# gergely-flamich/compression-without-quantization

Hardware: AMD Instinct MI355X
Metric: latent blocks encoded/s at KL=16 bits (higher is better)
Workload: dtype f32

## Files before the change

### compression_without_quantization_amd/csrc/cwq_kernels.hip

```cpp
#include <hip/hip_runtime.h>

#include <type_traits>
#include <stdint.h>

#include "cwq_device.h"
#include "cwq_kernels.h"

namespace cwq {

__global__ void __launch_bounds__(256) k_prep_dims(
    const float* __restrict__ t_scale, const float* __restrict__ p_loc,
    const float* __restrict__ p_scale, int64_t n, float nst, float sdiv, float rho,
    float* __restrict__ loc_s, float* __restrict__ scale_s, float* __restrict__ lognorm,
    float* __restrict__ out_sample, unsigned long long* __restrict__ keys, int64_t nb) {
  for (int64_t g = blockIdx.x * (int64_t)blockDim.x + threadIdx.x; g < nb;
       g += (int64_t)gridDim.x * blockDim.x)
    keys[g] = 0ull;
  for (int64_t i = blockIdx.x * (int64_t)blockDim.x + threadIdx.x; i < n;
       i += (int64_t)gridDim.x * blockDim.x) {
    float ls, ss;
    shard_consts(p_loc[i], p_scale[i], nst, sdiv, rho, ls, ss);
    loc_s[i] = ls;
    scale_s[i] = ss;
    lognorm[i] = lognorm_of(t_scale[i]);
    out_sample[i] = 0.0f;
  }
}

template <int DC, bool STEP0>
__device__ __forceinline__ float eval_row(const PhiloxStream& st, uint64_t kbase, int64_t d_rt,
                                          int align_rt, const float* __restrict__ loc_s,
                                          const float* __restrict__ scale_s,
                                          const float* __restrict__ mu,
                                          const float* __restrict__ sg,
                                          const float* __restrict__ lognorm,
                                          const float* __restrict__ best,
                                          const double* logtab) {
  return eval_row_f<DC>(st, kbase, d_rt, align_rt, logtab, [&](int64_t e, float zz) -> float {
    float s = scale_s[e] * zz;
    s = loc_s[e] + s;
    const float tv = STEP0 ? s : best[e] + s;
    return log_prob(tv, mu[e], sg[e], lognorm[e]);
  });
}

template <int DC, bool STEP0>
__global__ void __launch_bounds__(256) k_encode_eval(
    const float* __restrict__ t_loc, const float* __restrict__ t_scale,
    const float* __restrict__ loc_s, const float* __restrict__ scale_s,
    const float* __restrict__ lognorm, const float* __restrict__ best,
    const int64_t* __restrict__ block_off, int64_t ud, int64_t ntiles, int64_t tiles_per_block,
    int64_t cand_per_tile, int64_t n_cand, SeedSpec sd, int32_t step,
    unsigned long long* __restrict__ keys) {
  __shared__ double logtab[32];
  __shared__ unsigned long long wkey[4];
  fill_logtab(logtab);
  const uint32_t wv = wave_id();
  const uint32_t lane = threadIdx.x & 63u;

  for (int64_t tile = blockIdx.x; tile < ntiles; tile += gridDim.x) {
    const int64_t g = tile / tiles_per_block;
    const int64_t tt = tile - g * tiles_per_block;
    const BlockSpan sp = block_span(block_off, ud, g);
    const int64_t n0 = tt * cand_per_tile;
    const int64_t n1 = (n0 + cand_per_tile < n_cand) ? n0 + cand_per_tile : n_cand;
    const PhiloxStream st =
        generate_key(step_seed(sd.of(g), step), 42);
    const int align = (int)(((uint64_t)(n0 + wv) * (uint64_t)sp.d) & 3u);

    uint64_t bestk = 0;
    for (int64_t n = n0 + 4 * (int64_t)lane + wv; n < n1; n += 256) {
      const float v = eval_row<DC, STEP0>(st, (uint64_t)n * (uint64_t)sp.d, sp.d, align,
                                          loc_s + sp.off, scale_s + sp.off, t_loc + sp.off,
                                          t_scale + sp.off, lognorm + sp.off,
                                          STEP0 ? nullptr : best + sp.off, logtab);
      const uint64_t k = argmax_key(v, (uint32_t)n);
      bestk = k > bestk ? k : bestk;
    }
    bestk = wave_max_u64(bestk);
    if (lane == 0) wkey[wv] = bestk;
    __syncthreads();
    if (threadIdx.x == 0) {
      uint64_t m = wkey[0];
      for (int i = 1; i < 4; ++i) m = wkey[i] > m ? wkey[i] : m;
      if (m) atomicMax(&keys[g], (unsigned long long)m);
    }
    __syncthreads();
  }
}

constexpr float kPruneC1 = 0x1p-14f;
#ifndef CWQ_PRUNE_MIN_WAVES
#define CWQ_PRUNE_MIN_WAVES 6
#endif
#ifndef CWQ_XCD_BALANCE
#define CWQ_XCD_BALANCE 1
#endif
#ifndef CWQ_TAU_SHARE_MASK
#define CWQ_TAU_SHARE_MASK 15u
#endif
#ifndef CWQ_SURVIVOR_CAP
#define CWQ_SURVIVOR_CAP 1024
#endif

template <bool STEP0>
__device__ __forceinline__ float cand_diff(float z, float ls, float ss, float mu, float bb) {
  const float s = shard_sample(ls, ss, z);
  const float tv = STEP0 ? s : bb + s;
  return tv - mu;
}
__device__ __forceinline__ float lp_from_z(float z, float cc) {
  const float u = -0.5f * (z * z);
  return u - cc;
}


#ifdef CWQ_TILE_TIMES
constexpr int kTileTimes = 1 << 18;
__device__ unsigned long long g_tile_t0[kTileTimes], g_tile_t1[kTileTimes];
__device__ unsigned int g_tile_wg[kTileTimes];
#endif
#ifdef CWQ_PRUNE_STATS
__device__ unsigned long long g_prune_stats[72];
constexpr int kDbgBlocks = 1 << 20;
__device__ unsigned long long g_dbg_best[kDbgBlocks];
__device__ int g_seed_tau;
#endif

template <int D, bool STEP0, bool INTER>
__global__ void __launch_bounds__(256, CWQ_PRUNE_MIN_WAVES) k_encode_prune(
    const float* __restrict__ t_loc, const float* __restrict__ t_scale,
    const float* __restrict__ loc_s, const float* __restrict__ scale_s,
    const float* __restrict__ lognorm, const float* __restrict__ best, int64_t ntiles,
    int64_t tiles_per_block, int64_t cand_per_tile, int64_t n_cand, SeedSpec sd, int32_t step,
    int allow_screen, unsigned long long* __restrict__ keys, int64_t tail_from, int tail_div,
    uint32_t* __restrict__ tq) {
  static_assert(D % 8 == 0 && D >= 8 && D <= 64, "pruned path: D % 8 == 0, D <= 64");
  constexpr int G = D / 4;
  constexpr int NF = STEP0 ? 6 : 7;
  constexpr int NS = 2;
  __shared__ double logtab[32];
  __shared__ float4 cst[G * NF];
  __shared__ float4 scst[G * NS];
  __shared__ int2 meta[G];
  __shared__ float dscore[D];
  __shared__ float dA[D];
  __shared__ float dC[D];
  __shared__ float gscore[G];
  __shared__ int gpos[G];
  __shared__ float lowc;
  __shared__ float scr_a, scr_pq;
  __shared__ uint32_t tau_ord;
  __shared__ uint32_t sq_cnt;
  __shared__ uint32_t sq_n[CWQ_SURVIVOR_CAP];
  __shared__ float sq_ub[CWQ_SURVIVOR_CAP];
  __shared__ unsigned long long wkey[4];
  __shared__ uint32_t s_next;
#ifdef CWQ_PRUNE_STATS
  __shared__ uint32_t s_ps[72];
  for (int i = threadIdx.x; i < 72; i += blockDim.x) s_ps[i] = 0u;
#endif
  fill_logtab(logtab);
  const uint32_t wv = wave_id();
  const uint32_t lane = threadIdx.x & 63u;

  constexpr bool inter = INTER;
  const int64_t nbt = INTER ? ntiles / tiles_per_block : 0;
  auto next_tile = [&](int64_t cur) -> int64_t {
    if (tq == nullptr) return cur + gridDim.x;
    __syncthreads();
    if (threadIdx.x == 0) s_next = gridDim.x + atomicAdd(tq, 1u);
    __syncthreads();
    return (int64_t)s_next;
  };
  for (int64_t tile = blockIdx.x; tile < ntiles; tile = next_tile(tile)) {
    uint32_t tid = threadIdx.x;
    asm volatile("" : "+v"(tid));
#ifdef CWQ_TILE_TIMES
    if (tid == 0 && tile < kTileTimes) {
      g_tile_t0[tile] = __builtin_amdgcn_s_memrealtime();
      const uint32_t xcc = (uint32_t)__builtin_amdgcn_s_getreg((20) | (0 << 6) | ((4 - 1) << 11));
      g_tile_wg[tile] = (xcc << 24) | (blockIdx.x & 0xffffffu);
    }
#endif
    int64_t tord = tile;
    const int64_t treg = inter ? nbt * tail_from : 0;
    if (inter && CWQ_XCD_BALANCE && tq == nullptr && tile < treg && (treg & 7) == 0 &&
        (gridDim.x & 7u) == 0)
      tord = (tile & 7) * (treg >> 3) + (tile >> 3);
    const int64_t g = inter ? tord % nbt : tile / tiles_per_block;
    const int64_t tt = inter ? tord / nbt : tile - g * tiles_per_block;
    const int64_t off = g * D;
    int64_t n0, csz;
    if (tt < tail_from) {
      n0 = tt * cand_per_tile;
      csz = cand_per_tile;
    } else {
      csz = cand_per_tile / tail_div;
      n0 = tail_from * cand_per_tile + (tt - tail_from) * csz;
    }
    const int64_t n1 = (n0 + csz < n_cand) ? n0 + csz : n_cand;
    if (n0 >= n1) continue;
    const PhiloxStream st =
        generate_key(step_seed(sd.of(g), step), 42);

    if (tid < D) {
      const int j = tid;
      const float ls = loc_s[off + j], ss = scale_s[off + j], mu = t_loc[off + j];
      const float rs = 1.0f / t_scale[off + j];
      const float m = (STEP0 ? ls : best[off + j] + ls) - mu;
      float e = 0.5f * (ss * ss + m * m) * (rs * rs);
      dscore[j] = (e == e) ? e : -1.0f;
    }
    __syncthreads();
    if (tid < G) {
      const int q = tid;
      gscore[q] = ((dscore[4 * q] + dscore[4 * q + 1]) + dscore[4 * q + 2]) + dscore[4 * q + 3];
    }
    __syncthreads();
    if (tid < G) {
      const int q = tid;
      const float sq = gscore[q];
      int r = 0;
      for (int q2 = 0; q2 < G; ++q2) {
        const float s2 = gscore[q2];
        r += (s2 > sq || (s2 == sq && q2 < q)) ? 1 : 0;
      }
      gpos[q] = r;
      meta[r].x = q;
    }
    __syncthreads();
    int den_ok = 1, scr_ok = 1;
    if (tid < D) {
      const int j = tid, k = gpos[j >> 2], w = j & 3;
      float fj[7];
      const float sgj = t_scale[off + j];
      fj[0] = loc_s[off + j];
      fj[1] = scale_s[off + j];
      fj[2] = t_loc[off + j];
      fj[3] = sgj;
      fj[4] = lognorm[off + j];
      fj[5] = 1.0f / sgj;
      fj[6] = STEP0 ? 0.0f : best[off + j];
      float* c = reinterpret_cast<float*>(cst);
#pragma unroll
      for (int f = 0; f < NF; ++f) c[(k * NF + f) * 4 + w] = fj[f];
      den_ok = markstein_ok_den(sgj) ? 1 : 0;
      const ScreenDim o = screen_dim<STEP0>(fj[0], fj[1], fj[2], sgj, fj[4], fj[6]);
      float* sc = reinterpret_cast<float*>(scst);
      sc[(k * NS + 0) * 4 + w] = o.sa;
      sc[(k * NS + 1) * 4 + w] = o.sb;
      dA[j] = o.A;
      dC[j] = o.C;
      scr_ok = o.ok ? 1 : 0;
    }
    const bool fastdiv = __syncthreads_and(den_ok) != 0;
    const bool scr_all = __syncthreads_and(scr_ok) != 0;
    const bool screen = allow_screen && scr_all;
    if (tid <= G + 1) {
      const int kb = tid;
      const float* c = reinterpret_cast<const float*>(cst);
      double rf = 0.0, kk = 0.0, asum = 0.0, msum = 0.0, kall = 0.0, cvis = 0.0, a2 = 0.0,
             amax = 0.0;
#pragma unroll 1
      for (int p = 0; p < D; ++p) {
        const double mj = -(double)c[((p >> 2) * NF + 4) * 4 + (p & 3)];
        const double aj = __builtin_fabs(mj);
        asum += aj;
        msum += mj;
        kall += aj + mj;
        if (p >= 4 * kb) {
          rf += mj + 0x1p-17 * aj;
        } else {
          kk += aj + mj;
          if (screen) cvis += (double)dC[(meta[p >> 2].x << 2) + (p & 3)];
        }
        if (screen && kb == G + 1) {
          const double av = (double)dA[p];
          a2 += av * av;
          amax = av > amax ? av : amax;
        }
      }
      const double marg = 0x1p-20 * (__builtin_fabs(rf) + asum) + 0x1p-126;
      const double sl = 0x1p-14 * (__builtin_fabs(msum) + asum + kall) + 0x1p-126;
      if (kb <= G) {
        const float bk = screen ? round_up_f32(msum + cvis * (1.0 + 0x1p-20) + sl)
                                : round_up_f32(rf + 0x1p-14 * kk + marg);
        if (kb >= 1) meta[kb - 1].y = (int)f2u(bk);
        if (kb == G) lowc = round_up_f32(0x1p-14 * kk + marg);
      } else if (screen) {
        scr_a = screen_as(msum, sl, a2);
        scr_pq = screen_pq(amax, D);
      }
      if (kb == 0) {
        uint32_t t0 = ord_f32(-__builtin_inff());
        if (inter) {
          const unsigned long long kv =
              __hip_atomic_load(&keys[g], __ATOMIC_RELAXED, __HIP_MEMORY_SCOPE_AGENT);
          if ((uint32_t)(kv >> 32) > kArgmaxClampOrd) t0 = (uint32_t)(kv >> 32);
        }
        tau_ord = t0;
#ifdef CWQ_PRUNE_STATS
        if (g_seed_tau && g < kDbgBlocks && (g_dbg_best[g] >> 32) > kArgmaxClampOrd)
          tau_ord = (uint32_t)(g_dbg_best[g] >> 32);
#endif
        sq_cnt = 0u;
      }
    }
    __syncthreads();
    const float lc = lowc;
#ifdef CWQ_PRUNE_STATS
    const float tau_seed = unord_f32(tau_ord);
#endif
    const float sA = scr_a, sPq = scr_pq;

    const int64_t per_wave = (n1 - n0 + 3) / 4;
    const int64_t w0 = n0 + (int64_t)wv * per_wave;
    const uint32_t w1 = (uint32_t)((w0 + per_wave < n1) ? w0 + per_wave : n1);
    uint32_t wnext = (uint32_t)w0 + 64u;
    uint32_t n = (uint32_t)w0 + lane;
    int k = 0;
    float s = 0.0f;
#ifndef CWQ_TAU_FROM_KEYS
#define CWQ_TAU_FROM_KEYS 1
#endif
    float tau = (INTER && CWQ_TAU_FROM_KEYS) ? unord_f32(tau_ord) : -__builtin_inff();
#ifdef CWQ_PRUNE_STATS
    tau = tau_seed;
#endif
    uint64_t bestk = 0;
    uint32_t iter = 0;

    const PhiloxLo lok = philox_lo_key(st);
    auto pass = [&](auto screen_tag) {
      constexpr bool SCREEN = decltype(screen_tag)::value;
      for (;;) {
        const bool active = n < w1;
        if (__ballot(active) == 0ull) break;
        const int2 mt = meta[k];
        const uint32_t grp = (uint32_t)n * (uint32_t)G + (uint32_t)mt.x;
        const U4 x = philox10_lo(grp, lok, st.k0, st.k1);
        float z0, z1, z2, z3;
        float upper;
        if constexpr (SCREEN) {
          box_muller_screen(x.x, x.y, z0, z1);
          box_muller_screen(x.z, x.w, z2, z3);
          const float4* cq = scst + k * NS;
          const float4 sa = cq[0], sb = cq[1];
          const float a0 = __builtin_fmaf(sa.x, z0, sb.x);
          const float a1 = __builtin_fmaf(sa.y, z1, sb.y);
          const float a2 = __builtin_fmaf(sa.z, z2, sb.z);
          const float a3 = __builtin_fmaf(sa.w, z3, sb.w);
          s = __builtin_fmaf(-a0, a0, s);
          s = __builtin_fmaf(-a1, a1, s);
          s = __builtin_fmaf(-a2, a2, s);
          s = __builtin_fmaf(-a3, a3, s);
          upper = screen_row_upper(s, kScreenC1, u2f((uint32_t)mt.y));
        } else {
          box_muller_dev(x.x, x.y, logtab, z0, z1);
          box_muller_dev(x.z, x.w, logtab, z2, z3);
          const float4* cq = cst + k * NF;
          const float4 ls = cq[0], ss = cq[1], mu = cq[2], sg = cq[3], cc = cq[4], ry = cq[5];
          const float4 bb = STEP0 ? float4{0.f, 0.f, 0.f, 0.f} : cq[6];
          const float d0 = cand_diff<STEP0>(z0, ls.x, ss.x, mu.x, bb.x);
          const float d1 = cand_diff<STEP0>(z1, ls.y, ss.y, mu.y, bb.y);
          const float d2 = cand_diff<STEP0>(z2, ls.z, ss.z, mu.z, bb.z);
          const float d3 = cand_diff<STEP0>(z3, ls.w, ss.w, mu.w, bb.w);
          float y0 = div_rn_markstein(d0, sg.x, ry.x);
          float y1 = div_rn_markstein(d1, sg.y, ry.y);
          float y2 = div_rn_markstein(d2, sg.z, ry.z);
          float y3 = div_rn_markstein(d3, sg.w, ry.w);
          const bool ok = fastdiv & markstein_ok4(d0, d1, d2, d3);
          if (__builtin_expect(__ballot(!ok) != 0ull, 0)) {
            if (!ok) {
              y0 = d0 / sg.x;
              y1 = d1 / sg.y;
              y2 = d2 / sg.z;
              y3 = d3 / sg.w;
            }
          }
          s = s + lp_from_z(y0, cc.x);
          s = s + lp_from_z(y1, cc.y);
          s = s + lp_from_z(y2, cc.z);
          s = s + lp_from_z(y3, cc.w);
          upper = (s + __builtin_fabsf(s) * kPruneC1) + u2f((uint32_t)mt.y);
        }
        k += 1;
        const bool complete = (k == G);
        const bool below = upper < tau;
#ifdef CWQ_PRUNE_STATS
        const bool prune = !complete && below;
#endif
        const bool done = complete || below || !active;
        const uint64_t m = __ballot(complete) | __ballot(below) |
                           (__builtin_amdgcn_read_exec() & ~__ballot(active));
        if (complete && active && upper >= tau) {
          float lower;
          if constexpr (SCREEN)
            lower = screen_row_lower(s, kScreenC2, sA, sPq);
          else
            lower = (s - __builtin_fabsf(s) * kPruneC1) - lc;
          tau = fmaxf(tau, lower);
          const uint32_t slot = atomicAdd(&sq_cnt, 1u);
          if (slot < CWQ_SURVIVOR_CAP) {
            sq_n[slot] = (uint32_t)n;
            sq_ub[slot] = upper;
          } else {
#ifdef CWQ_PRUNE_STATS
            atomicAdd(&g_prune_stats[69], 1ull);
#endif
            const float v = eval_row<D, STEP0>(st, (uint64_t)n * D, D, 0, loc_s + off,
                                               scale_s + off, t_loc + off, t_scale + off,
                                               lognorm + off, STEP0 ? nullptr : best + off, logtab);
            const uint64_t kv = argmax_key(v, (uint32_t)n);
            bestk = kv > bestk ? kv : bestk;
          }
        }
#ifdef CWQ_PRUNE_STATS
        if (active && (complete || prune)) atomicAdd(&s_ps[k], 1u);
        if (active && complete) atomicAdd(&s_ps[65], 1u);
        if (active && complete && upper >= tau) atomicAdd(&s_ps[66], 1u);
#endif
        const uint32_t rank = __builtin_amdgcn_mbcnt_hi((uint32_t)(m >> 32),
                                                        __builtin_amdgcn_mbcnt_lo((uint32_t)m, 0u));
        if (done) {
          n = wnext + rank;
          k = 0;
          s = 0.0f;
        }
        wnext += (uint32_t)__builtin_popcountll(m);
        if (((++iter) & CWQ_TAU_SHARE_MASK) == 0u) {
          const float tm = wave_max_f32(tau);
          if (lane == 0) atomicMax(&tau_ord, ord_f32(tm));
          tau = fmaxf(tau, unord_f32(__atomic_load_n(&tau_ord, __ATOMIC_RELAXED)));
        }
      }
    };
#ifdef CWQ_PRUNE_STATS
    if (screen && tid == 0) atomicAdd(&g_prune_stats[67], 1ull);
#endif
    if (screen)
      pass(std::true_type{});
    else
      pass(std::false_type{});

    {
      const float tm = wave_max_f32(tau);
      if (lane == 0) atomicMax(&tau_ord, ord_f32(tm));
    }
    __syncthreads();
    const float tau_final = unord_f32(tau_ord);
    const uint32_t nsurv = sq_cnt < CWQ_SURVIVOR_CAP ? sq_cnt : CWQ_SURVIVOR_CAP;
    for (uint32_t i = tid; i < nsurv; i += blockDim.x) {
      if (sq_ub[i] >= tau_final) {
#ifdef CWQ_PRUNE_STATS
        atomicAdd(&g_prune_stats[68], 1ull);
#endif
        const uint32_t nn = sq_n[i];
        const float v = eval_row<D, STEP0>(st, (uint64_t)nn * D, D, 0, loc_s + off,
                                           scale_s + off, t_loc + off, t_scale + off,
                                           lognorm + off, STEP0 ? nullptr : best + off, logtab);
        const uint64_t kv = argmax_key(v, nn);
        bestk = kv > bestk ? kv : bestk;
      }
    }

    bestk = wave_max_u64(bestk);
    if (lane == 0) wkey[wv] = bestk;
    __syncthreads();
    if (tid == 0) {
      uint64_t mk = wkey[0];
      for (int i = 1; i < 4; ++i) mk = wkey[i] > mk ? wkey[i] : mk;
      if (mk) atomicMax(&keys[g], (unsigned long long)mk);
#ifdef CWQ_PRUNE_STATS
      if (!g_seed_tau && g < kDbgBlocks) g_dbg_best[g] = mk;
#endif
#ifdef CWQ_TILE_TIMES
      if (tile < kTileTimes) g_tile_t1[tile] = __builtin_amdgcn_s_memrealtime();
#endif
    }
#ifdef CWQ_PRUNE_STATS
    if (tid < 72) {
      if (s_ps[tid]) atomicAdd(&g_prune_stats[tid], (unsigned long long)s_ps[tid]);
      s_ps[tid] = 0u;
    }
#endif
    __syncthreads();
  }
}

__device__ __forceinline__ double block_sum_d(double v, double* red) {
  red[threadIdx.x] = v;
  __syncthreads();
  for (int w = 128; w > 0; w >>= 1) {
    if ((int)threadIdx.x < w) red[threadIdx.x] += red[threadIdx.x + w];
    __syncthreads();
  }
  const double r = red[0];
  __syncthreads();
  return r;
}

__host__ __device__ __forceinline__ int64_t csr_cls_stride(int64_t d) { return (d + 6) / 4 + 1; }
constexpr int64_t kCsrSortUnits = 2048;

template <bool STEP0>
__global__ void __launch_bounds__(256) k_csr_prep(
    const float* __restrict__ t_loc, const float* __restrict__ t_scale,
    const float* __restrict__ loc_s, const float* __restrict__ scale_s,
    const float* __restrict__ lognorm, const float* __restrict__ best,
    const int64_t* __restrict__ block_off, int64_t ud, int64_t nb, float2* __restrict__ sab,
    float* __restrict__ cdim, float* __restrict__ bpre, uint32_t* __restrict__ ordu,
    float4* __restrict__ grp, uint32_t* __restrict__ gtau, float4* __restrict__ abp,
    int64_t lds_dims, int64_t coop_min_d) {
  __shared__ double red[5][4];
  __shared__ double wscan[4];
  __shared__ double ucs[256];
  __shared__ unsigned long long skey[kCsrSortUnits];
  const int tid = threadIdx.x;
  const int lane = tid & 63, wv = tid >> 6;
  const bool lead = blockIdx.y == 0;
  for (int64_t g = blockIdx.x; g < nb; g += gridDim.x) {
    const BlockSpan sp = block_span(block_off, ud, g);
    const int64_t off = sp.off, d = sp.d;
    ScreenSums u;
    float2* sabg = sab + off + 8 * g + 4;
    float* cg = cdim + off;
    if (lead && tid < 8) {
      if (tid < 4) sabg[tid - 4] = float2{0.f, 0.f};
      sabg[d + tid] = float2{0.f, 0.f};
    }
    for (int64_t j = tid; j < d; j += 256) {
      const ScreenDim o =
          screen_dim<STEP0>(loc_s[off + j], scale_s[off + j], t_loc[off + j], t_scale[off + j],
                            lognorm[off + j], STEP0 ? 0.0f : best[off + j]);
      sabg[j] = float2{o.sa, o.sb};
      cg[j] = o.C;
      u.add(o);
    }
    u.sm = wave_sum_f64(u.sm);
    u.sa = wave_sum_f64(u.sa);
    u.sk = wave_sum_f64(u.sk);
    u.s2 = wave_sum_f64(u.s2);
    u.mx = wave_max_f64(u.mx);
    if (lane == 0) {
      red[0][wv] = u.sm;
      red[1][wv] = u.sa;
      red[2][wv] = u.sk;
      red[3][wv] = u.s2;
      red[4][wv] = u.mx;
    }
    __threadfence_block();
    const bool all_ok = __syncthreads_and(u.ok) != 0;
    ScreenSums S;
    S.sm = ((red[0][0] + red[0][1]) + red[0][2]) + red[0][3];
    S.sa = ((red[1][0] + red[1][1]) + red[1][2]) + red[1][3];
    S.sk = ((red[2][0] + red[2][1]) + red[2][2]) + red[2][3];
    S.s2 = ((red[3][0] + red[3][1]) + red[3][2]) + red[3][3];
    S.mx = red[4][0];
    for (int w = 1; w < 4; ++w) S.mx = red[4][w] > S.mx ? red[4][w] : S.mx;
    const bool coop_blk = d >= coop_min_d;
    const ScreenBlock bc =
        screen_block_consts(S, d, coop_blk ? 16.0 + (double)d / 64.0 : (double)d);
    const double SM = S.sm, sl = bc.sl;
    const int64_t reg = off + 12 * g, cs = csr_cls_stride(d);
    const bool recs = abp != nullptr && d > lds_dims;
    auto sab_at = [&](int64_t j) {
      const unsigned long long v = __hip_atomic_load(
          reinterpret_cast<unsigned long long*>(sabg + j), __ATOMIC_RELAXED,
          __HIP_MEMORY_SCOPE_AGENT);
      return float2{u2f((uint32_t)v), u2f((uint32_t)(v >> 32))};
    };
    for (int c = (int)blockIdx.y; c < 4; c += (int)gridDim.y) {
      auto unit = [&](int64_t u, double& csum, double& gain) {
        csum = 0.0;
        gain = 0.0;
        for (int t = 0; t < 4; ++t) {
          const int64_t j = 4 * u - c + t;
          if (j >= 0 && j < d) {
            const float2 ab = sab_at(j);
            const float xc = u2f(__hip_atomic_load(reinterpret_cast<uint32_t*>(cg + j),
                                                   __ATOMIC_RELAXED, __HIP_MEMORY_SCOPE_AGENT));
            csum += (double)xc;
            gain += (double)ab.x * (double)ab.x * (0.5 / 0.6931471805599453) +
                    (double)ab.y * (double)ab.y - (double)xc;
          }
        }
      };
      auto key_of = [&](int64_t u) {
        double cu, gu;
        unit(u, cu, gu);
        const float gf = (float)(gu > 0.0 ? gu : 0.0);
        return ((unsigned long long)ord_f32(gf) << 32) | (0xffffffffull - (uint64_t)u);
      };
      const int64_t U = (d + c + 3) / 4;
      const bool sorted = all_ok && U <= kCsrSortUnits;
      const bool small = U <= 256;
      if (sorted && small) {
        unsigned long long key = 0ull;
        if (tid < U) {
          double cu, gu;
          unit(tid, cu, gu);
          ucs[tid] = cu;
          const float gf = (float)(gu > 0.0 ? gu : 0.0);
          key = ((unsigned long long)ord_f32(gf) << 32) | (0xffffffffull - (uint64_t)tid);
          skey[tid] = key;
        }
        __syncthreads();
        int r = 0;
        if (tid < U)
          for (int i = 0; i < (int)U; ++i) r += skey[i] > key ? 1 : 0;
        __syncthreads();
        if (tid < U) skey[r] = key;
        __syncthreads();
      } else if (sorted) {
        int64_t P = 1;
        while (P < U) P <<= 1;
        for (int64_t u = tid; u < P; u += 256) skey[u] = u < U ? key_of(u) : 0ull;
        __syncthreads();
        for (int64_t k = 2; k <= P; k <<= 1) {
          for (int64_t jj = k >> 1; jj > 0; jj >>= 1) {
            for (int64_t i = tid; i < P; i += 256) {
              const int64_t l = i ^ jj;
              if (l > i) {
                const unsigned long long x = skey[i], y = skey[l];
                const bool desc = (i & k) == 0;
                if (desc ? (x < y) : (x > y)) {
                  skey[i] = y;
                  skey[l] = x;
                }
              }
            }
            __syncthreads();
          }
        }
      }
      double carry = 0.0;
      for (int64_t base = 0; base <= U; base += 256) {
        const int64_t k = base + tid;
        int64_t u = k;
        if (sorted && k < U) u = (int64_t)(0xffffffffull - (skey[k] & 0xffffffffull));
        double cu = 0.0, gu;
        if (all_ok && k < U) {
          if (sorted && small)
            cu = ucs[u];
          else
            unit(u, cu, gu);
        }
        if (recs && k <= U) {
          float e[8];
          for (int t = 0; t < 4; ++t) {
            const int64_t j = 4 * u - c + t;
            float2 ab = float2{0.f, 0.f};
            if (k < U && j >= 0 && j < d) ab = sab_at(j);
            e[2 * t] = ab.x;
            e[2 * t + 1] = ab.y;
          }
          float4* rr = abp + 2 * (csr_rec_base(off) + c * cs + k);
          rr[0] = float4{e[0], e[1], e[2], e[3]};
          rr[1] = float4{e[4], e[5], e[6], e[7]};
        }
        double v = cu;
#pragma unroll
        for (int o = 1; o < 64; o <<= 1) {
          const double t = __shfl_up(v, (unsigned)o, 64);
          if (lane >= o) v += t;
        }
        if (lane == 63) wscan[wv] = v;
        __syncthreads();
        double pre = 0.0;
        for (int w = 0; w < wv; ++w) pre += wscan[w];
        const double total = ((wscan[0] + wscan[1]) + wscan[2]) + wscan[3];
        const double excl = carry + (pre + v) - cu;
        if (k <= U) {
          bpre[reg + c * cs + k] = round_up_f32(SM + excl * (1.0 + 0x1p-20) + sl);
          ordu[reg + c * cs + k] = (uint32_t)(k < U ? u : U);
        }
        carry += total;
        __syncthreads();
      }
    }
    if (lead && tid == 0) {
      grp[g] = (all_ok && bc.finite && d > 0) ? float4{bc.c1, bc.c2, bc.as, bc.pq}
                                              : float4{0.f, 0.f, 0.f, 0.f};
      gtau[g * CWQ_CSR_GTAU_STRIDE] = ord_f32(-__builtin_inff());
    }
    __syncthreads();
  }
}

constexpr int kRowChunk = 248;

template <bool STEP0>
__device__ __forceinline__ float exact_row_wave(
    const PhiloxStream& st, uint64_t kbase, int64_t d, const float* __restrict__ loc_s,
    const float* __restrict__ scale_s, const float* __restrict__ mu,
    const float* __restrict__ sg, const float* __restrict__ lognorm,
    const float* __restrict__ best, const double* logtab, float* buf, uint32_t lane) {
  const int64_t vec = d & ~(int64_t)7;
  float acc = 0.0f;
  for (int64_t j0 = 0; j0 < d; j0 += kRowChunk) {
    const int64_t cnt = (d - j0) < kRowChunk ? d - j0 : kRowChunk;
    const uint64_t k0 = kbase + (uint64_t)j0;
    const uint64_t blk = (k0 >> 2) + lane;
    const int64_t ef = (int64_t)(blk << 2) - (int64_t)k0;
    if (ef < cnt) {
      const F4 z = normal4_dev(st, blk, logtab);
#pragma unroll
      for (int t = 0; t < 4; ++t) {
        const int64_t e = ef + t;
        if (e >= 0 && e < cnt) {
          const int64_t j = j0 + e;
          const float zz = t == 0 ? z.a : (t == 1 ? z.b : (t == 2 ? z.c : z.d));
          float v = scale_s[j] * zz;
          v = loc_s[j] + v;
          const float tv = STEP0 ? v : best[j] + v;
          buf[e] = log_prob(tv, mu[j], sg[j], lognorm[j]);
        }
      }
    }
    __builtin_amdgcn_fence(__ATOMIC_SEQ_CST, "wavefront");
    __builtin_amdgcn_wave_barrier();
    if (lane < 8) {
      for (int64_t e = lane; e < cnt && j0 + e < vec; e += 8) acc = acc + buf[e];
    } else if (lane == 8) {
      for (int64_t e = (vec > j0 ? vec - j0 : 0); e < cnt; ++e) acc = acc + buf[e];
    }
    __builtin_amdgcn_fence(__ATOMIC_SEQ_CST, "wavefront");
    __builtin_amdgcn_wave_barrier();
  }
  float p[8];
#pragma unroll
  for (int l = 0; l < 8; ++l) p[l] = __shfl(acc, l, 64);
  return eigen_fold8(p, __shfl(acc, 8, 64));
}

template <bool STEP0>
__global__ void __launch_bounds__(256) k_encode_rows_wave(
    const float* __restrict__ t_loc, const float* __restrict__ t_scale,
    const float* __restrict__ loc_s, const float* __restrict__ scale_s,
    const float* __restrict__ lognorm, const float* __restrict__ best,
    const int64_t* __restrict__ block_off, int64_t ud, int64_t nb, int n_bits, SeedSpec sd,
    int32_t step, unsigned long long* __restrict__ keys) {
  __shared__ double logtab[32];
  __shared__ float rowbuf[4][kRowChunk];
  __shared__ unsigned long long wkey[4];
  __shared__ int64_t wblk[4];
  fill_logtab(logtab);
  const uint32_t wv = wave_id();
  const uint32_t lane = threadIdx.x & 63u;
  const int64_t rows = nb << n_bits;
  const int64_t cmask = ((int64_t)1 << n_bits) - 1;
  for (int64_t r0 = 4 * (int64_t)blockIdx.x; r0 < rows; r0 += 4 * (int64_t)gridDim.x) {
    const int64_t r = r0 + wv;
    uint64_t k = 0;
    int64_t g = -1;
    if (r < rows) {
      g = r >> n_bits;
      const int64_t n = r & cmask;
      const BlockSpan sp = block_span(block_off, ud, g);
      if (sp.d > 0) {
        const PhiloxStream st = generate_key(step_seed(sd.of(g), step), 42);
        const float v = exact_row_wave<STEP0>(
            st, (uint64_t)n * (uint64_t)sp.d, sp.d, loc_s + sp.off, scale_s + sp.off,
            t_loc + sp.off, t_scale + sp.off, lognorm + sp.off,
            STEP0 ? nullptr : best + sp.off, logtab, rowbuf[wv], lane);
// ... 2442 lines not shown
```

Baseline: 3.249 million.

## Cooperatively score survivors per wave and pack screen records for scalar-indexed pruning loop

The survivor re-evaluation pass now compacts qualifying candidates within each wave and scores up to eight rows at once. Lanes split each row's dimensions, stage log-probs in a per-wave LDS buffer and reduce them with shuffles, replacing one full serial row evaluation per lane. The pruning loop tracks group offsets instead of row indices, uses byte offsets into a packed 48-byte VisitRec holding screen coefficients and bounds, and uses fcmp ballot and asm pins to keep values in scalar registers. The aim is to cut divergence and serial work in survivor scoring and to trim instruction overhead in the hot loop, at the cost of extra LDS and per-row integer division on survivors.

```diff
diff --git a/compression_without_quantization_amd/csrc/cwq_kernels.hip b/compression_without_quantization_amd/csrc/cwq_kernels.hip
--- a/compression_without_quantization_amd/csrc/cwq_kernels.hip
+++ b/compression_without_quantization_amd/csrc/cwq_kernels.hip
@@ -115,6 +115,48 @@
 }
 
 
+struct VisitRec {
+  float4 sa, sb;
+  int grp;
+  int bk;
+  int pad[2];
+};
+static_assert(sizeof(VisitRec) == 48, "VisitRec: 48 bytes");
+
+template <int D, bool STEP0>
+__device__ __forceinline__ float score_rows_wave(
+    const PhiloxStream& st, const uint32_t* rows, uint32_t cnt, const float* __restrict__ loc_s,
+    const float* __restrict__ scale_s, const float* __restrict__ mu,
+    const float* __restrict__ sg, const float* __restrict__ lognorm,
+    const float* __restrict__ best, const double* logtab, float* buf, uint32_t lane) {
+  constexpr uint32_t G = D / 4;
+  const uint32_t r = lane / G, u = lane - r * G;
+  if (r < cnt) {
+    const F4 z = normal4_dev(st, (uint64_t)rows[r] * G + u, logtab);
+#pragma unroll
+    for (int t = 0; t < 4; ++t) {
+      const uint32_t j = 4u * u + (uint32_t)t;
+      const float zz = t == 0 ? z.a : (t == 1 ? z.b : (t == 2 ? z.c : z.d));
+      float v = scale_s[j] * zz;
+      v = loc_s[j] + v;
+      const float tv = STEP0 ? v : best[j] + v;
+      buf[r * D + j] = log_prob(tv, mu[j], sg[j], lognorm[j]);
+    }
+  }
+  __builtin_amdgcn_fence(__ATOMIC_SEQ_CST, "wavefront");
+  __builtin_amdgcn_wave_barrier();
+  float acc = 0.0f;
+  const uint32_t fr = lane >> 3;
+  if (fr < cnt)
+    for (uint32_t e = lane & 7u; e < (uint32_t)D; e += 8u) acc = acc + buf[fr * D + e];
+  __builtin_amdgcn_fence(__ATOMIC_SEQ_CST, "wavefront");
+  __builtin_amdgcn_wave_barrier();
+  float p[8];
+#pragma unroll
+  for (int l = 0; l < 8; ++l) p[l] = __shfl(acc, (int)((lane & ~7u) + (uint32_t)l), 64);
+  return eigen_fold8(p, 0.0f);
+}
+
 #ifdef CWQ_TILE_TIMES
 constexpr int kTileTimes = 1 << 18;
 __device__ unsigned long long g_tile_t0[kTileTimes], g_tile_t1[kTileTimes];
@@ -138,11 +180,12 @@
   static_assert(D % 8 == 0 && D >= 8 && D <= 64, "pruned path: D % 8 == 0, D <= 64");
   constexpr int G = D / 4;
   constexpr int NF = STEP0 ? 6 : 7;
-  constexpr int NS = 2;
+  constexpr int RW = (64 / G) < 8 ? (64 / G) : 8;
   __shared__ double logtab[32];
   __shared__ float4 cst[G * NF];
-  __shared__ float4 scst[G * NS];
+  __shared__ VisitRec vrec[G];
   __shared__ int2 meta[G];
+  __shared__ float rowbuf[4][RW * D];
   __shared__ float dscore[D];
   __shared__ float dA[D];
   __shared__ float dC[D];
@@ -228,6 +271,7 @@
       }
       gpos[q] = r;
       meta[r].x = q;
+      vrec[r].grp = q;
     }
     __syncthreads();
     int den_ok = 1, scr_ok = 1;
@@ -247,9 +291,9 @@
       for (int f = 0; f < NF; ++f) c[(k * NF + f) * 4 + w] = fj[f];
       den_ok = markstein_ok_den(sgj) ? 1 : 0;
       const ScreenDim o = screen_dim<STEP0>(fj[0], fj[1], fj[2], sgj, fj[4], fj[6]);
-      float* sc = reinterpret_cast<float*>(scst);
-      sc[(k * NS + 0) * 4 + w] = o.sa;
-      sc[(k * NS + 1) * 4 + w] = o.sb;
+      float* sc = reinterpret_cast<float*>(&vrec[k]);
+      sc[w] = o.sa;
+      sc[4 + w] = o.sb;
       dA[j] = o.A;
       dC[j] = o.C;
       scr_ok = o.ok ? 1 : 0;
@@ -286,7 +330,10 @@
       if (kb <= G) {
         const float bk = screen ? round_up_f32(msum + cvis * (1.0 + 0x1p-20) + sl)
                                 : round_up_f32(rf + 0x1p-14 * kk + marg);
-        if (kb >= 1) meta[kb - 1].y = (int)f2u(bk);
+        if (kb >= 1) {
+          meta[kb - 1].y = (int)f2u(bk);
+          vrec[kb - 1].bk = (int)f2u(bk);
+        }
         if (kb == G) lowc = round_up_f32(0x1p-14 * kk + marg);
       } else if (screen) {
         scr_a = screen_as(msum, sl, a2);
@@ -316,11 +363,11 @@
 
     const int64_t per_wave = (n1 - n0 + 3) / 4;
     const int64_t w0 = n0 + (int64_t)wv * per_wave;
-    const uint32_t w1 = (uint32_t)((w0 + per_wave < n1) ? w0 + per_wave : n1);
-    uint32_t wnext = (uint32_t)w0 + 64u;
-    uint32_t n = (uint32_t)w0 + lane;
-    int k = 0;
-    float s = 0.0f;
+    const int64_t w1 = (w0 + per_wave < n1) ? w0 + per_wave : n1;
+    const uint32_t w0g =
+        (uint32_t)__builtin_amdgcn_readfirstlane((int)((uint32_t)w0 * (uint32_t)G));
+    const uint32_t ng_end = (uint32_t)__builtin_amdgcn_readfirstlane(
+        (int)(w1 > w0 ? (uint32_t)(w1 - w0) * (uint32_t)G : 0u));
 #ifndef CWQ_TAU_FROM_KEYS
 #define CWQ_TAU_FROM_KEYS 1
 #endif
@@ -329,24 +376,38 @@
     tau = tau_seed;
 #endif
     uint64_t bestk = 0;
-    uint32_t iter = 0;
 
     const PhiloxLo lok = philox_lo_key(st);
     auto pass = [&](auto screen_tag) {
       constexpr bool SCREEN = decltype(screen_tag)::value;
-      for (;;) {
-        const bool active = n < w1;
-        if (__ballot(active) == 0ull) break;
-        const int2 mt = meta[k];
-        const uint32_t grp = (uint32_t)n * (uint32_t)G + (uint32_t)mt.x;
-        const U4 x = philox10_lo(grp, lok, st.k0, st.k1);
+      constexpr uint32_t KS = SCREEN ? (uint32_t)sizeof(VisitRec) : 1u;
+      uint32_t ng = lane * (uint32_t)G;
+      uint32_t wnext_g = 64u * (uint32_t)G;
+      uint32_t kp = 0;
+      float s = 0.0f;
+      uint32_t iter = 0;
+      bool active = ng < ng_end;
+      uint64_t m_act = __builtin_amdgcn_ballot_w64(active);
+      while (m_act != 0ull) {
+        int2 mt;
+        float4 sa, sb;
+        if constexpr (SCREEN) {
+          const char* rp = reinterpret_cast<const char*>(vrec) + kp;
+          sa = *reinterpret_cast<const float4*>(rp);
+          sb = *reinterpret_cast<const float4*>(rp + 16);
+          mt = *reinterpret_cast<const int2*>(rp + 32);
+        } else {
+          mt = meta[kp];
+        }
+        const uint32_t grp = (ng + (uint32_t)mt.x) + w0g;
+        uint32_t pk0 = st.k0, pk1 = st.k1;
+        asm volatile("" : "+s"(pk0), "+s"(pk1));
+        const U4 x = philox10_lo(grp, lok, pk0, pk1);
         float z0, z1, z2, z3;
         float upper;
         if constexpr (SCREEN) {
           box_muller_screen(x.x, x.y, z0, z1);
           box_muller_screen(x.z, x.w, z2, z3);
-          const float4* cq = scst + k * NS;
-          const float4 sa = cq[0], sb = cq[1];
           const float a0 = __builtin_fmaf(sa.x, z0, sb.x);
           const float a1 = __builtin_fmaf(sa.y, z1, sb.y);
           const float a2 = __builtin_fmaf(sa.z, z2, sb.z);
@@ -359,7 +420,7 @@
         } else {
           box_muller_dev(x.x, x.y, logtab, z0, z1);
           box_muller_dev(x.z, x.w, logtab, z2, z3);
-          const float4* cq = cst + k * NF;
+          const float4* cq = cst + kp * NF;
           const float4 ls = cq[0], ss = cq[1], mu = cq[2], sg = cq[3], cc = cq[4], ry = cq[5];
           const float4 bb = STEP0 ? float4{0.f, 0.f, 0.f, 0.f} : cq[6];
           const float d0 = cand_diff<STEP0>(z0, ls.x, ss.x, mu.x, bb.x);
@@ -385,16 +446,23 @@
           s = s + lp_from_z(y3, cc.w);
           upper = (s + __builtin_fabsf(s) * kPruneC1) + u2f((uint32_t)mt.y);
         }
-        k += 1;
-        const bool complete = (k == G);
+        kp += KS;
+        const bool complete = (kp == KS * (uint32_t)G);
         const bool below = upper < tau;
+        const bool reach = SCREEN ? !below : (upper >= tau);
 #ifdef CWQ_PRUNE_STATS
         const bool prune = !complete && below;
+        const uint32_t k = kp / KS;
 #endif
         const bool done = complete || below || !active;
-        const uint64_t m = __ballot(complete) | __ballot(below) |
-                           (__builtin_amdgcn_read_exec() & ~__ballot(active));
-        if (complete && active && upper >= tau) {
+        uint64_t m = __builtin_amdgcn_ballot_w64(complete) |
+                     __builtin_amdgcn_fcmpf(upper, tau, 4 ) |
+                     (__builtin_amdgcn_read_exec() & ~m_act);
+        asm volatile("" : "+s"(m));
+        if (__builtin_expect(complete && active && reach, 0)) {
+          uint32_t ngc = ng;
+          asm volatile("" : "+v"(ngc));
+          const uint32_t n = (w0g + ngc) / (uint32_t)G;
           float lower;
           if constexpr (SCREEN)
             lower = screen_row_lower(s, kScreenC2, sA, sPq);
@@ -424,16 +492,18 @@
         const uint32_t rank = __builtin_amdgcn_mbcnt_hi((uint32_t)(m >> 32),
                                                         __builtin_amdgcn_mbcnt_lo((uint32_t)m, 0u));
         if (done) {
-          n = wnext + rank;
-          k = 0;
+          ng = wnext_g + rank * (uint32_t)G;
+          kp = 0;
           s = 0.0f;
         }
-        wnext += (uint32_t)__builtin_popcountll(m);
+        wnext_g += (uint32_t)__builtin_popcountll(m) * (uint32_t)G;
         if (((++iter) & CWQ_TAU_SHARE_MASK) == 0u) {
           const float tm = wave_max_f32(tau);
           if (lane == 0) atomicMax(&tau_ord, ord_f32(tm));
           tau = fmaxf(tau, unord_f32(__atomic_load_n(&tau_ord, __ATOMIC_RELAXED)));
         }
+        active = ng < ng_end;
+        m_act = __builtin_amdgcn_ballot_w64(active);
       }
     };
 #ifdef CWQ_PRUNE_STATS
@@ -451,17 +521,34 @@
     __syncthreads();
     const float tau_final = unord_f32(tau_ord);
     const uint32_t nsurv = sq_cnt < CWQ_SURVIVOR_CAP ? sq_cnt : CWQ_SURVIVOR_CAP;
-    for (uint32_t i = tid; i < nsurv; i += blockDim.x) {
-      if (sq_ub[i] >= tau_final) {
+    const uint32_t nsurv_u = (uint32_t)__builtin_amdgcn_readfirstlane((int)nsurv);
+    const uint32_t sl = tid & 63u;
+    for (uint32_t c0 = wv * 64u; c0 < nsurv_u; c0 += 256u) {
+      const uint32_t i = c0 + sl;
+      const bool q = i < nsurv_u && sq_ub[i] >= tau_final;
+      const uint32_t nn = i < nsurv_u ? sq_n[i] : 0u;
+      const uint64_t qm = __builtin_amdgcn_ballot_w64(q);
+      if (qm == 0ull) continue;
 #ifdef CWQ_PRUNE_STATS
-        atomicAdd(&g_prune_stats[68], 1ull);
-#endif
-        const uint32_t nn = sq_n[i];
-        const float v = eval_row<D, STEP0>(st, (uint64_t)nn * D, D, 0, loc_s + off,
-                                           scale_s + off, t_loc + off, t_scale + off,
-                                           lognorm + off, STEP0 ? nullptr : best + off, logtab);
-        const uint64_t kv = argmax_key(v, nn);
-        bestk = kv > bestk ? kv : bestk;
+      if (q) atomicAdd(&g_prune_stats[68], 1ull);
+#endif
+      const uint32_t qr = __builtin_amdgcn_mbcnt_hi((uint32_t)(qm >> 32),
+                                                    __builtin_amdgcn_mbcnt_lo((uint32_t)qm, 0u));
+      __builtin_amdgcn_fence(__ATOMIC_SEQ_CST, "wavefront");
+      __builtin_amdgcn_wave_barrier();
+      if (q) sq_n[c0 + qr] = nn;
+      __builtin_amdgcn_fence(__ATOMIC_SEQ_CST, "wavefront");
+      __builtin_amdgcn_wave_barrier();
+      const uint32_t qn = (uint32_t)__builtin_popcountll(qm);
+      for (uint32_t b = 0; b < qn; b += (uint32_t)RW) {
+        const uint32_t cnt = qn - b < (uint32_t)RW ? qn - b : (uint32_t)RW;
+        const float v = score_rows_wave<D, STEP0>(
+            st, sq_n + c0 + b, cnt, loc_s + off, scale_s + off, t_loc + off, t_scale + off,
+            lognorm + off, STEP0 ? nullptr : best + off, logtab, rowbuf[wv], sl);
+        if ((sl & 7u) == 0u && (sl >> 3) < cnt) {
+          const uint64_t kv = argmax_key(v, sq_n[c0 + b + (sl >> 3)]);
+          bestk = kv > bestk ? kv : bestk;
+        }
       }
     }
 
```

New measurement: 3.491 million, median of 6. 1.07x the previous value.
